# orybkin/video-gcp

Measured on AMD Instinct MI355X. Metric: predicted frames/sec, 64x64x3 seq_len=80 gcp_tree (posterior forward + all loss terms, model(inputs) and model.loss() of train.py:157-159, batch-stat BatchNorm), higher is better.
Workload: dtype f32 (encoder / decoder convs and the tree GEMMs from 512 rows: split-f16 MFMA with f32 accumulate, f32-equivalent; everything else exact f32 MFMA)

## Files before the change

### include/gcpx.h

```cpp
#ifndef GCPX_H
#define GCPX_H

#include <stdint.h>

#ifdef __cplusplus
extern "C" {
#endif

#define GCPX_VERSION 1

typedef enum gcpx_status {
    GCPX_OK = 0,
    GCPX_ERR_INVALID_ARG = -1,
    GCPX_ERR_UNSUPPORTED = -2,
    GCPX_ERR_HIP = -3,
    GCPX_ERR_COMM = -4
} gcpx_status;

typedef enum gcpx_act { GCPX_ACT_NONE = 0, GCPX_ACT_LRELU = 1, GCPX_ACT_TANH = 2 } gcpx_act;

int gcpx_version(void);
const char* gcpx_last_error(void);
int gcpx_conv_grid(void);

// ... 36 lines not shown
    const int32_t* raw_row_map;
    const int32_t* src_row_map;
    const int32_t* src_row_frames;
    int32_t n_src_rows;
    int32_t w_split_log2;
    const void* wpk_split;
    const int32_t* w_split_log2_dev;
    int32_t split_layout;
    int32_t nll_rows;
    const float* nll_target;
    float* nll_partial;
    const float* nll_row_weight;
    float nll_scale;
    int32_t _pad3;
    float* images_rows;
    int64_t images_rows_dup;
    const float* bwd_r;
    const float *bwd_scale, *bwd_shift, *bwd_mean, *bwd_rstd;
    const float* addend;
    int32_t addend_frame_div;
    int32_t _pad4;
} gcpx_conv_args;

typedef enum gcpx_split_layout { GCPX_SPLIT_PLAIN = 0, GCPX_SPLIT_ROWFOLD = 1, GCPX_SPLIT_HEAD32 = 2 } gcpx_split_layout;

int gcpx_conv3x3(const gcpx_conv_args* a, void* stream);
int gcpx_conv3x3_grid(const gcpx_conv_args* a);
int gcpx_conv4x4s2(const gcpx_conv_args* a, void* stream);
int gcpx_conv4x4s2_grid(void);
int gcpx_conv4x4s2_image(const float* x, const float* wpk, const float* bias, float* out,
                         int32_t F, int32_t Hin, int32_t Win, int32_t Cout, int32_t out_act, void* stream);

int gcpx_bn_finalize(const float* partial, int32_t n_partial, int32_t pitch, int32_t C, double count,
                     const float* gamma, const float* beta, float eps, float* scale, float* shift,
                     float* running_mean, float* running_var, float momentum, float* mean_out, float* rstd_out,
                     void* stream);
int gcpx_randn(float* out, int64_t n, uint64_t* state, void* stream);
int gcpx_bn_fold(const float* running_mean, const float* running_var, const float* gamma, const float* beta,
                 float eps, int32_t C, float* scale, float* shift, void* stream);

typedef struct gcpx_row_src {
    const float* ptr;
    const int32_t* rowidx;
    const float* scale;
    const float* shiftv;
    int64_t sb, sr;
    int32_t width;
// ... 510 lines not shown
```

### video-gcp_amd/csrc/conv3x3.hip

```cpp
#include "common.h"

#include <type_traits>

int gcpx_launch_up16_split(const gcpx_conv_args* a, hipStream_t stream, int grid);
int gcpx_launch_up32_split(const gcpx_conv_args* a, hipStream_t stream, int which, int grid);
int gcpx_launch_up16_fold(const gcpx_conv_args* a, hipStream_t stream, int grid);
int gcpx_launch_wave_split(const gcpx_conv_args* a, hipStream_t stream, int ct, int depth);

namespace {

template <int TILE> struct TileShape;
template <> struct TileShape<0> { static constexpr int TH = 8, TW = 32, TF = 1; };
template <> struct TileShape<1> { static constexpr int TH = 16, TW = 16, TF = 1; };
template <> struct TileShape<2> { static constexpr int TH = 8, TW = 8, TF = 4; };
template <> struct TileShape<3> { static constexpr int TH = 8, TW = 16, TF = 1; };

template <bool UP, int CC, int CT, int TILE>
struct ConvCfg {
    using TS = TileShape<TILE>;
    static constexpr int TH = TS::TH, TW = TS::TW, TF = TS::TF;
    static constexpr int RH = TH + 2, RW = TW + 2;
    static constexpr int LH = TH / 2 + 2, LW = TW / 2 + 2;
    static constexpr int CCP = (CC == 16) ? 24 : CC + 4;
    static constexpr int C4 = CC / 4;
    static constexpr int HI_FLOATS = TF * RH * RW * CCP;
    static constexpr int RAW_FLOATS = UP ? TF * LH * LW * CC : 0;
    static constexpr int RED_FLOATS = 4 * 2 * CT * 16;
    static constexpr int LDS_BYTES = (HI_FLOATS + RAW_FLOATS) * 4;
    static constexpr int PR = TH * TW * TF / 64;
// ... 1013 lines not shown
                red[(wave * 2 + 0) * 16 + q * 4 + r] = s1;
                red[(wave * 2 + 1) * 16 + q * 4 + r] = s2;
            }
        }
        __syncthreads();
        if (tid < 32) {
            const int which = tid >> 4, c = tid & 15;
            float sum = 0.f;
#pragma unroll
            for (int w = 0; w < 8; ++w) sum += red[(w * 2 + which) * 16 + c];
            a.stats_partial[((size_t)blockIdx.x * 2 + which) * 16 + c] = sum;
        }
    }
}

int launch_up16(const gcpx_conv_args* a, hipStream_t stream, bool query_only) {
    const int nchunk = a->Cin / 16;
    const int lds = UpWaveCfg::lds_bytes(nchunk);
    int grid = gcpx_conv_grid() / 2;
    const int nitems = a->F * (a->Hout / 4) * (a->Wout / 16);
    if (!a->stats_partial && grid * 8 > nitems) grid = (nitems + 7) / 8;
    if (query_only) return grid;
    if (a->wpk_split && a->split_layout == GCPX_SPLIT_ROWFOLD) return gcpx_launch_up16_fold(a, stream, grid);
    if (a->wpk_split) return gcpx_launch_up16_split(a, stream, grid);
    static int lds_set = 0;
    if (lds > lds_set) {
        hipError_t e = hipFuncSetAttribute(reinterpret_cast<const void*>(conv3x3_up16_kernel),
                                           hipFuncAttributeMaxDynamicSharedMemorySize, lds);
        if (e != hipSuccess) {
            gcpx_set_error("conv3x3 up16: hipFuncSetAttribute(%d B LDS): %s", lds, hipGetErrorString(e));
            return GCPX_ERR_HIP;
        }
        lds_set = lds;
    }
    const int ipw = (nitems + grid * 8 - 1) / (grid * 8);
    hipLaunchKernelGGL(conv3x3_up16_kernel, dim3(grid), dim3(512), lds, stream, *a, ipw, nitems);
    GCPX_CHECK_LAUNCH();
    return GCPX_OK;
}

int g_conv_grid = 0;

template <bool UP, int CC, int CT, int TILE>
int launch(const gcpx_conv_args* a, hipStream_t stream, bool query_only = false) {
    using Cfg = ConvCfg<UP, CC, CT, TILE>;
    if (a->Hout % Cfg::TH || a->Wout % Cfg::TW) {
// ... 40 lines not shown
int gcpx_launch_head_split(const gcpx_conv_args* a, hipStream_t stream);

static int conv3x3_dispatch(const gcpx_conv_args* a, hipStream_t stream, bool query_only) {
    GCPX_CHECK_ARG(a != nullptr, "null args");
    GCPX_CHECK_ARG(a->nsrc == 1 || a->nsrc == 2, "nsrc must be 1 or 2");
    GCPX_CHECK_ARG(a->src[0].C % 16 == 0 && (a->nsrc == 1 || a->src[1].C % 16 == 0), "source channels must be multiples of 16");
    const bool leading = !a->upsample && a->nsrc == 1 && a->Cin < a->src[0].C && a->Cin >= 32 && a->Cin % 16 == 0 && a->Cout == 16 && a->wpk_split &&
                         a->split_layout == GCPX_SPLIT_PLAIN && (!a->src_row_map || a->src_row_frames) && !getenv("GCPX_DGRAD_TILED");
    GCPX_CHECK_ARG(leading || a->Cin == a->src[0].C + (a->nsrc == 2 ? a->src[1].C : 0), "Cin != sum of sources");
    GCPX_CHECK_ARG(a->wpk && a->bias, "weights/bias missing");
    GCPX_CHECK_ARG(a->F > 0, "F <= 0");
    if (a->upsample) GCPX_CHECK_ARG(a->Hout == 2 * a->Hin && a->Wout == 2 * a->Win, "upsample: Hout != 2*Hin");
    else GCPX_CHECK_ARG(a->Hout == a->Hin && a->Wout == a->Win, "no upsample: Hout != Hin");
    const int CT = (a->Cout + 15) / 16;
    const bool need_out = a->head_mode == GCPX_HEAD_RAW || a->head_mode == GCPX_HEAD_DLM_BOTH;
    GCPX_CHECK_ARG(!need_out || a->out, "out is NULL");
    GCPX_CHECK_ARG(need_out || a->images, "images is NULL");
    GCPX_CHECK_ARG(!need_out || a->out_pitch % 4 == 0, "out_pitch % 4");
    GCPX_CHECK_ARG(!a->images_rows || (a->wpk_split && a->raw_row_map && a->images && a->Cout == 100 && !a->upsample &&
                                       (a->head_mode == GCPX_HEAD_DLM_MEAN || a->head_mode == GCPX_HEAD_DLM_BOTH ||
                                        a->head_mode == GCPX_HEAD_DLM_NLL || a->head_mode == GCPX_HEAD_DLM_NLL_GRAD)),
                   "images_rows: split-f16 mixture head with raw_row_map and images only");
    const int W = a->Wout;
    GCPX_CHECK_ARG(!a->addend || (a->upsample && a->addend_frame_div > 0 && a->wpk_split && a->Cout != 16),
                   "addend: split-f16 upsampling blocks with 32 / 64 output channels, addend_frame_div > 0");
    if (!a->upsample) {
        GCPX_CHECK_ARG(a->nsrc == 1 && a->src[0].frame_div == 1, "non-upsampling 3x3 conv takes one per-frame source");
        if (a->Cin == 16 && !a->src_row_map && W % 16 == 0 && a->Hout % 4 == 0) {
            if (a->Cout == 100) {
                GCPX_CHECK_ARG(!need_out || a->out_pitch >= 100, "mixture head: out_pitch < 100");
                GCPX_CHECK_ARG(a->head_mode != GCPX_HEAD_DLM_NLL || a->wpk_split, "GCPX_HEAD_DLM_NLL is built for the split-f16 head (wpk_split)");
                if (a->wpk_split) return query_only ? gcpx_conv_grid() / 2 : gcpx_launch_head_split(a, stream);
                return query_only ? gcpx_conv_grid() / 2 : launch_head<6, true>(a, stream);
            }
            if (CT == 1) return query_only ? gcpx_conv_grid() / 2 : launch_head<1, false>(a, stream);
        }
        GCPX_CHECK_ARG(a->head_mode == GCPX_HEAD_RAW && (!a->stats_partial || a->bwd_r), "plain 3x3 conv stores raw output, no statistics");
        if (a->bwd_r) {
            const bool fits = a->wpk_split && a->split_layout == GCPX_SPLIT_PLAIN && W % 16 == 0 && a->Hout % 4 == 0 && a->Cout == 16 &&
                              a->out_pitch == 16 && a->Cin >= 32 && a->Cin % 16 == 0 && (!a->src_row_map || a->src_row_frames) &&
                              a->stats_partial && a->bwd_scale && a->bwd_shift && a->bwd_mean && a->bwd_rstd && !getenv("GCPX_DGRAD_TILED");
            GCPX_CHECK_ARG(fits, "bwd_r: split-f16 plain 3x3 conv, 16 output channels at pitch 16, Cin >= 32, stats_partial and the four BatchNorm vectors");
        }
        static const bool tiled_only = getenv("GCPX_DGRAD_TILED") != nullptr;
        static const int depth = getenv("GCPX_DGRAD_DEPTH") ? atoi(getenv("GCPX_DGRAD_DEPTH")) : 2;
        GCPX_CHECK_ARG(!a->src_row_frames || (a->src_row_map && a->n_src_rows >= 0), "src_row_frames needs src_row_map and n_src_rows");
        if (!tiled_only && W % 16 == 0 && a->Hout % 4 == 0 && a->Cout == 16 && a->out_pitch % 4 == 0 && CT == 1 && a->Cin >= 32 &&
            (!a->src_row_map || a->src_row_frames) && WaveCfg<1>::lds_bytes(a->Cin / 16) <= 152 * 1024) {
// ... 8 lines not shown
        GCPX_CHECK_ARG(!leading, "Cin < src[0].C is built for the 16-output-channel wave kernel only (W % 16 == 0, H % 4 == 0)");
        static const bool wave32 = getenv("GCPX_DGRAD_NOWAVE32") == nullptr;
        if (wave32 && !tiled_only && W % 16 == 0 && a->Hout % 4 == 0 && a->Cout == 32 && a->out_pitch % 4 == 0 && a->Cin % 16 == 0 &&
            (!a->src_row_map || a->src_row_frames) && WaveCfg<2>::lds_bytes(a->Cin / 16) <= 152 * 1024) {
            if (query_only) return gcpx_conv_grid() / 2;
            if (a->wpk_split && a->split_layout == GCPX_SPLIT_PLAIN) {
                const int st = gcpx_launch_wave_split(a, stream, 2, 1);
                if (st != -1) return st;
            }
            return launch_wave<2, 1>(a, stream);
        }
        const int tile = W >= 32 ? 0 : (W == 16 ? 1 : (W == 8 ? 2 : -1));
#define GCPX_PLAIN(CC_, CT_)                                                            \
        do {                                                                            \
            if (tile == 0) return launch<false, CC_, CT_, 0>(a, stream, query_only);    \
            if (tile == 1) return launch<false, CC_, CT_, 1>(a, stream, query_only);    \
            if (tile == 2) return launch<false, CC_, CT_, 2>(a, stream, query_only);    \
        } while (0)
        if (a->Cin % 16 == 0 && CT == 4) GCPX_PLAIN(16, 4);
        if (a->Cin % 16 == 0 && CT == 2) GCPX_PLAIN(16, 2);
        if (a->Cin % 16 == 0 && CT == 1) GCPX_PLAIN(16, 1);
#undef GCPX_PLAIN
    } else {
        GCPX_CHECK_ARG(a->Cin % 32 == 0, "upsampling 3x3 conv expects Cin % 32 == 0");
        GCPX_CHECK_ARG(a->head_mode == GCPX_HEAD_RAW, "decoder blocks store raw output");
        if (a->Cout == 16) {
            GCPX_CHECK_ARG(W % 16 == 0 && a->Hout % 4 == 0 && a->out_pitch == 16 && a->Cin <= 64, "16-channel block shape");
            return launch_up16(a, stream, query_only);
        }
        if (a->wpk_split && !query_only && a->Cout == CT * 16 && a->out_pitch == a->Cout && a->out_act == GCPX_ACT_NONE) {
            if (W == 16 && CT == 2) return gcpx_launch_up32_split(a, stream, 0, launch<true, 32, 2, 1>(a, stream, true));
            if (W == 8 && CT == 2) return gcpx_launch_up32_split(a, stream, 1, launch<true, 32, 2, 2>(a, stream, true));
            if (W == 8 && CT == 4) return gcpx_launch_up32_split(a, stream, 2, launch<true, 32, 4, 2>(a, stream, true));
        }
        GCPX_CHECK_ARG(query_only || !a->addend, "addend: split-f16 upsampling blocks with 32 / 64 output channels only");
        if (W == 16 && CT == 2) return launch<true, 32, 2, 1>(a, stream, query_only);
        if (W == 8 && CT == 2) return launch<true, 32, 2, 2>(a, stream, query_only);
        if (W == 8 && CT == 4) return launch<true, 32, 4, 2>(a, stream, query_only);
    }
    gcpx_set_error("conv3x3: unsupported shape (up=%d Cin=%d Cout=%d W=%d)", a->upsample, a->Cin, a->Cout, W);
    return GCPX_ERR_UNSUPPORTED;
}

extern "C" int gcpx_conv3x3(const gcpx_conv_args* a, void* stream_) {
    return conv3x3_dispatch(a, reinterpret_cast<hipStream_t>(stream_), false);
}

// ... 2 lines not shown
```

### video-gcp_amd/csrc/conv3x3_split.hip

```cpp
#include "common.h"
#include "split_mfma.h"

#include <cstdlib>
#include <type_traits>

namespace {

struct SplitUpCfg {
    static constexpr int RW = 18, RH = 6, LW = 10, LH = 4, CC = 16, KS = 5;
    static constexpr int RAW_BYTES = LH * LW * CC * 4;
    static constexpr int PLANE_BYTES = RH * RW * 32;
    static constexpr int WAVE_BYTES = RAW_BYTES + 2 * PLANE_BYTES;
    static constexpr int NS = (LH * LW * 4 + 63) / 64;
    static constexpr int W_CHUNK_BYTES = KS * 2 * 1024;
    static int lds_bytes(int nchunk) { return nchunk * W_CHUNK_BYTES + 8 * WAVE_BYTES + 8 * 2 * 16 * 4; }
};

__global__ void __launch_bounds__(512, 2) conv3x3_up16_split_kernel(const gcpx_conv_args a, const int items_per_wave,
                                                                    const int nitems) {
    using Cfg = SplitUpCfg;
    constexpr int RW = Cfg::RW, RH = Cfg::RH, LW = Cfg::LW, LH = Cfg::LH, CC = Cfg::CC, NS = Cfg::NS, KS = Cfg::KS;
    extern __shared__ float4 smem4[];
    const int nchunk = a.Cin / CC;
    const char* wl = reinterpret_cast<const char*>(smem4);
// ... 748 lines not shown
    }
    if (optr) store_out();
    if (a.stats_partial) {
#pragma unroll
        for (int r = 0; r < 4; ++r) {
            const float s1 = row16_sum(st1[r]);
            const float s2 = row16_sum(st2[r]);
            if (j == 0) {
                red[(wave * 2 + 0) * 16 + q * 4 + r] = s1;
                red[(wave * 2 + 1) * 16 + q * 4 + r] = s2;
            }
        }
        __syncthreads();
        if (tid < 32) {
            const int which = tid >> 4, c = tid & 15;
            float sum = 0.f;
#pragma unroll
            for (int w = 0; w < 8; ++w) sum += red[(w * 2 + which) * 16 + c];
            a.stats_partial[((size_t)blockIdx.x * 2 + which) * 16 + c] = sum;
        }
    }
}

typedef unsigned int u32x4s __attribute__((ext_vector_type(4)));

template <int CT>
struct WaveSplitCfg {
    static constexpr int RW = 18, RH = 6, KS = 5;
    static constexpr int PLANE_BYTES = RH * RW * 32;
    static constexpr int REGION_BYTES = 2 * PLANE_BYTES;
    static constexpr int W_CHUNK_BYTES = KS * CT * 2 * 1024;
    static constexpr int NS = (RH * RW * 4 + 63) / 64;
    static int lds_bytes(int nchunk) { return nchunk * W_CHUNK_BYTES + 8 * REGION_BYTES + 256 + 1024; }
};

template <int CT, int DEPTH, bool ACTB = false>
__global__ void __launch_bounds__(512, 2) conv3x3_wave_split_kernel(const gcpx_conv_args a, const int nitems) {
    using Cfg = WaveSplitCfg<CT>;
    constexpr int RW = Cfg::RW, RH = Cfg::RH, NS = Cfg::NS, KS = Cfg::KS;
    extern __shared__ float4 smem4[];
    const int nchunk = a.Cin / 16;
    const char* wl = reinterpret_cast<const char*>(smem4);
    const int tid = threadIdx.x, lane = tid & 63;
    const int wave = __builtin_amdgcn_readfirstlane(tid >> 6);
    char* reg = reinterpret_cast<char*>(smem4) + nchunk * Cfg::W_CHUNK_BYTES + wave * Cfg::REGION_BYTES;
    const int j = lane & 15, q = lane >> 4;
// ... 347 lines not shown
    GCPX_CHECK_ARG(a->Cin == 32 && a->Cout == 16 && a->Hin % Cfg::R == 0 && a->Hout == 2 * a->Hin && a->Wout == 2 * a->Win && a->Wout % 16 == 0,
                   "row-folded block: 32 -> 16 channels, Hin a multiple of 4, output width a multiple of 16");
    GCPX_CHECK_ARG(a->src[0].C % 4 == 0 && (a->nsrc == 1 ? a->src[0].C == 32 : a->src[0].C + a->src[1].C == 32), "source channels");
    static const bool prio = getenv("GCPX_FOLD_NOPRIO") == nullptr;
    auto kern = prio ? conv3x3_up16_fold_kernel<true> : conv3x3_up16_fold_kernel<false>;
    static bool attr_set = false;
    if (!attr_set) {
        for (auto k : {conv3x3_up16_fold_kernel<true>, conv3x3_up16_fold_kernel<false>}) {
            hipError_t e = hipFuncSetAttribute(reinterpret_cast<const void*>(k), hipFuncAttributeMaxDynamicSharedMemorySize, Cfg::LDS_BYTES);
            if (e != hipSuccess) {
                gcpx_set_error("conv3x3 row-folded up16: hipFuncSetAttribute(%d B LDS): %s", Cfg::LDS_BYTES, hipGetErrorString(e));
                return GCPX_ERR_HIP;
            }
        }
        attr_set = true;
    }
    const int nitems = a->F * (a->Hin / Cfg::R) * (a->Wout / 16);
    const int ipw = (nitems + grid * 8 - 1) / (grid * 8);
    hipLaunchKernelGGL(kern, dim3(grid), dim3(512), Cfg::LDS_BYTES, stream, *a, ipw, nitems);
    GCPX_CHECK_LAUNCH();
    return GCPX_OK;
}

extern "C" int gcpx_fold_upsample_weights(const float* w, int32_t Cout, int32_t Cin, float* out, void* stream_) {
    GCPX_CHECK_ARG(w && out && Cout > 0 && Cin > 0, "bad arguments");
    const int n = 24 * Cout * Cin;
    hipLaunchKernelGGL(fold_up_weights_kernel, dim3((n + 255) / 256), dim3(256), 0, reinterpret_cast<hipStream_t>(stream_), w, Cout, Cin, out);
    GCPX_CHECK_LAUNCH();
    return GCPX_OK;
}

int gcpx_launch_wave_split(const gcpx_conv_args* a, hipStream_t stream, int ct, int depth) {
    const int nchunk = a->Cin / 16;
    if (ct == 1) {
        if (WaveSplitCfg<1>::lds_bytes(nchunk) > 160 * 1024) return -1;
        if (a->bwd_r) {
            static const int d = getenv("GCPX_WAVE_DEPTH") ? atoi(getenv("GCPX_WAVE_DEPTH")) : 1;
            return d == 3 ? launch_wave_split_t<1, 3, true>(a, stream) : d == 2 ? launch_wave_split_t<1, 2, true>(a, stream) : launch_wave_split_t<1, 1, true>(a, stream);
        }
        return depth == 2 ? launch_wave_split_t<1, 2>(a, stream) : launch_wave_split_t<1, 1>(a, stream);
    }
    if (WaveSplitCfg<2>::lds_bytes(nchunk) > 160 * 1024) return -1;
    return launch_wave_split_t<2, 1>(a, stream);
}
```

### video-gcp_amd/forward_plan.py

```python
import ctypes as C
import os
from contextlib import contextmanager

import torch

from . import packing as pk
from . import runtime as rt
from .hparams import GCPHParams
from .params import init_params, encoder_layers, encoder_skip_layers, decoder_layers
from .plan_ops import _Plan, _addr, N_LANES


class ForwardPlanMixin:

    def _plan_encoder(self, plan, tag, x_ptr, F, out_ptr, out_ob, out_orow, out_rpb):
        hp, P, lib = self._hp, self.pk, self.lib
        G = lib.gcpx_conv4x4s2_grid()
        S = hp.img_sz
        skip_idx = encoder_skip_layers(hp)
        skips = {}
        a0 = self._buf(f"{tag}.a0", (F, S // 2, S // 2, hp.ngf))
        enc_rec = dict(F=F, x_ptr=x_ptr, a0=a0, r={}, out=(out_ptr, out_ob, out_orow, out_rpb))
        plan.rec[f"enc:{tag}"] = enc_rec
        plan.add(f"enc.input:{tag}", lib.gcpx_conv4x4s2_image, x_ptr, P["enc.input.w"].data_ptr(),
# ... 70 lines not shown
    def _plan_decoder_features(self, plan, e_src, F, rpb, skips):
        hp, P, lib = self._hp, self.pk, self.lib
        ctop = self._c_top
        d0 = self._buf("dec.d0", (F, 4, 4, ctop))
        plan.rec["dec"] = dict(F=F, rpb=rpb, e_src=e_src, d0=d0, blocks=[], skips=skips)
        nrb = lib.gcpx_gemm_row_blocks(F, 16 * ctop)
        st = self._buf("dec.st0", (nrb, 2, 16 * ctop)) if self.training else None
        self._gemm(plan, "dec.input", [e_src], F, 16 * ctop, rpb, P["dec.input.w"], P["dec.input.b"], out=d0.data_ptr(),
                   ob=rpb * 16 * ctop, orow=16 * ctop, stats=st)
        sc, sh = self._bn(plan, "dec.bn0", "decoder.net.input.norm", ctop, st, nrb, 16 * ctop, F * 16)
        prev = (d0.data_ptr(), ctop, 1, sc, sh, rt.ACT_LRELU)
        res = 4
        for name, c_prev, c_skip, skip_idx, cout in decoder_layers(hp):
            srcs = [prev]
            if skip_idx >= 0:
                t, C_, ssc, ssh, sact = skips[skip_idx]
                assert C_ == c_skip and t.shape[1] == res
                srcs.append((t.data_ptr(), C_, rpb, ssc, ssh, sact))
            o = self._buf(f"dec.{name}", (F, 2 * res, 2 * res, cout))
            cpad = (cout + 15) // 16 * 16
            hoist = (skip_idx >= 0 and rpb > 1 and F % rpb == 0 and self.split_f16 and cout in (32, 64) and c_prev % 32 == 0 and
                     c_skip % 32 == 0 and f"dec.{name}" in self.pk_split and "fold" not in self.pk_split[f"dec.{name}"] and
                     os.environ.get("GCPX_NO_SKIP_HOIST") is None)
            addend = None
            if hoist:
                addend = self._buf(f"dec.{name}.skip", (F // rpb, 2 * res, 2 * res, cout))
                t, C_, ssc, ssh, sact = skips[skip_idx]
                zb = self._buf(f"dec.{name}.zero_bias", (cpad,), zero=True)
                a_s = self._conv_args([(t.data_ptr(), C_, 1, ssc, ssh, sact)], F // rpb, res, res, 2 * res, 2 * res, cout, cout,
                                      P[f"dec.{name}.w"], zb, addend, upsample=1)
                self._set_split(a_s, f"dec.{name}")
                a_s.wpk_split = a_s.wpk_split + (c_prev // 32) * 9 * (cpad // 16) * 2048
                plan.keep.append(a_s)
                plan.add(f"dec.{name}.skip", lib.gcpx_conv3x3, C.byref(a_s))
                srcs_main = [prev]
            else:
                srcs_main = srcs
            a = self._conv_args(srcs_main, F, res, res, 2 * res, 2 * res, cout, cout, P[f"dec.{name}.w"], P[f"dec.{name}.b"],
                                o, upsample=1, stats=(o if self.training else None))
            if hoist:
                a.addend, a.addend_frame_div = addend.data_ptr(), rpb
            self._set_split(a, f"dec.{name}")
            Gl = lib.gcpx_conv3x3_grid(C.byref(a))
            assert Gl > 0, rt.lib().gcpx_last_error()
            st = self._buf(f"dec.st.{name}", (Gl, 2, cpad)) if self.training else None
            a.stats_partial = st.data_ptr() if st is not None else None
            plan.keep.append(a)
            plan.add(f"dec.{name}", lib.gcpx_conv3x3, C.byref(a))
            plan.rec["dec"]["blocks"].append(dict(name=name, srcs=srcs, out=o, res_in=res, cout=cout, c_prev=c_prev, c_skip=c_skip,
                                                  skip_idx=skip_idx))
            res *= 2
            sc, sh = self._bn(plan, f"dec.bn.{name}", f"decoder.net.{name}.norm", cout, st, Gl, cpad, F * res * res)
            prev = (o.data_ptr(), cout, 1, sc, sh, rt.ACT_LRELU)
        assert res == hp.img_sz
        return prev

    def _build_plan(self, key, tin):
        hp, P, lib = self._hp, self.pk, self.lib
        B, has_traj, has_z, sample_prior, phase = key[0], key[1], key[2], key[3], key[4]
        pred_len = key[9]
        train_aux = has_traj and phase == "train" and not sample_prior
        L, T, N = hp.hierarchy_levels, hp.max_seq_len, hp.n_nodes
        nz, nv, H, SD = hp.nz_enc, hp.nz_vae, hp.nz_mid_lstm, hp.lstm_state_dim
        PS = 2 ** L + 1
        plan = _Plan(lib)
# ... 463 lines not shown
```

### video-gcp_amd/packing.py

```python
import torch

_LANE = torch.arange(64)
_LI = _LANE % 16
_LQ = _LANE // 16


def _pad_rows(w, rows):
    if w.shape[0] == rows:
        return w
    pad = torch.zeros((rows - w.shape[0],) + tuple(w.shape[1:]), dtype=w.dtype, device=w.device)
    return torch.cat([w, pad], 0)


def pack_gemm(w):
    N, K = w.shape
    assert K % 16 == 0, (N, K)
    NT = (N + 15) // 16
    w = _pad_rows(w, NT * 16)
    dev = w.device
    kg = torch.arange(K // 16, device=dev)[:, None, None, None]
    nt = torch.arange(NT, device=dev)[None, :, None, None]
    li = _LI.to(dev)[None, None, :, None]
    lq = _LQ.to(dev)[None, None, :, None]
    s = torch.arange(4, device=dev)[None, None, None, :]
# ... 297 lines not shown
    return torch.stack(out, 0).float()


def conv3x3_fold_gather(fw):
    assert fw.shape == (24, 16, 32)
    dev = fw.device
    t = torch.arange(24, device=dev)[:, None, None]
    li = _LI.to(dev)[None, :, None]
    lq = _LQ.to(dev)[None, :, None]
    el = torch.arange(8, device=dev)[None, None, :]
    return fw[t, li, lq * 8 + el].contiguous()


def pack_conv3x3_fold(w):
    w1, w2, e = split_f16(conv3x3_fold_gather(fold_up_weights(w)))
    return torch.stack([w1, w2], 1).contiguous().view(torch.int16), e


def conv3x3_fold_index():
    ids = torch.arange(24 * 16 * 32, dtype=torch.float64).view(24, 16, 32)
    return conv3x3_fold_gather(ids).reshape(-1).to(torch.int32)


def lstm_gate_interleave(w_ih, w_hh, b_ih, b_hh):
    H = w_hh.shape[1]
    w = torch.cat([w_ih, w_hh], dim=1)
    K = w.shape[1]
    w = w.view(4, H, K).permute(1, 0, 2).reshape(4 * H, K)
    b = (b_ih + b_hh).view(4, H).t().reshape(4 * H)
    return w.contiguous(), b.contiguous()
```

### video-gcp_amd/runtime.py

```python
import ctypes as C
import os

_HERE = os.path.dirname(os.path.abspath(__file__))
LIB_PATH = os.path.join(_HERE, "libgcpx.so")

ACT_NONE, ACT_LRELU, ACT_TANH = 0, 1, 2
HEAD_RAW, HEAD_DLM_MEAN, HEAD_DLM_BOTH, HEAD_TANH_NCHW, HEAD_DLM_NLL, HEAD_DLM_NLL_GRAD = 0, 1, 2, 3, 4, 5
SPLIT_PLAIN, SPLIT_ROWFOLD, SPLIT_HEAD32 = 0, 1, 2
EPI_NONE, EPI_LRELU, EPI_LSTM, EPI_GAUSS_SAMPLE = 0, 1, 2, 3
MLP_PLAIN, MLP_GAUSS, MLP_TANH = 0, 1, 2

vp = C.c_void_p
i32 = C.c_int32
i64 = C.c_int64


class ConvSrc(C.Structure):
    _fields_ = [("ptr", vp), ("scale", vp), ("shift", vp), ("C", i32), ("frame_div", i32), ("act", i32), ("_pad", i32)]


class ConvArgs(C.Structure):
    _fields_ = [("src", ConvSrc * 2), ("nsrc", i32), ("F", i32), ("Hin", i32), ("Win", i32), ("Hout", i32),
                ("Wout", i32), ("Cin", i32), ("Cout", i32), ("out_pitch", i32), ("upsample", i32), ("out_act", i32),
                ("head_mode", i32), ("wpk", vp), ("bias", vp), ("out", vp), ("images", vp), ("stats_partial", vp),
                ("raw_row_map", vp), ("src_row_map", vp), ("src_row_frames", vp), ("n_src_rows", i32), ("w_split_log2", i32), ("wpk_split", vp), ("w_split_log2_dev", vp),
                ("split_layout", i32), ("nll_rows", i32), ("nll_target", vp), ("nll_partial", vp), ("nll_row_weight", vp),
                ("nll_scale", C.c_float), ("_pad3", i32), ("images_rows", vp), ("images_rows_dup", i64), ("bwd_r", vp), ("bwd_scale", vp), ("bwd_shift", vp), ("bwd_mean", vp),
                ("bwd_rstd", vp), ("addend", vp), ("addend_frame_div", i32), ("_pad4", i32)]


class LossArgs(C.Structure):
# ... 281 lines not shown
```

### video-gcp_amd/weights.py

```python
import ctypes as C
import os
from contextlib import contextmanager

import torch

from . import packing as pk
from . import runtime as rt
from .hparams import GCPHParams
from .params import init_params, encoder_layers, encoder_skip_layers, decoder_layers
from .plan_ops import _addr


class WeightsMixin:

    def _flatten_params(self, params):
        off, self._poff = 0, {}
        for k, v in params.items():
            self._poff[k] = (off, tuple(v.shape))
            off += (v.numel() + 3) // 4 * 4
        self.theta = torch.zeros(off, dtype=torch.float32, device=self.device)
        self.sd = {}
        for k, v in params.items():
            o, shp = self._poff[k]
            view = self.theta[o:o + v.numel()].view(shp)
# ... 21 lines not shown
            d["gn_b"] = torch.stack([sd[f"{prefix}.pyramid-{i}.norm.bias"] for i in range(n_mid)]).contiguous()
        d["w_out"] = pk.pack_gemm(sd[f"{prefix}.head.linear.weight"])
        d["b_out"] = pk.pad_vec(sd[f"{prefix}.head.linear.bias"], out_pad)
        return d

    def _pack_all(self):
        if self._arena is not None:
            self.repack()
            return
        self.pk = self._pack_tree(self.sd)
        if self._hp.tree_lstm:
            self._pack_fused_embed()
        self._pack_split()
        self._pack_gemm_split()

    def _pack_split(self):
        self.pk_split = {}
        hp = self._hp
        todo = []
        if hp.decoder_distribution == "discrete_logistic_mixture":
            todo.append(("dec.head", "decoder.gen_head.conv.weight", pk.dlm_channel_perm(hp.n_mixtures)))
            if self.head32 and hp.n_mixtures == 10 and hp.head_channels == 100:
                todo.append(("dec.head32", "decoder.gen_head.conv.weight", ("head32", pk.dlm_channel_perm(hp.n_mixtures))))
        for name, c_prev, c_skip, skip_idx, cout in decoder_layers(hp):
            if cout == 16 and c_prev + c_skip == 32:
                todo.append((f"dec.{name}", f"decoder.net.{name}.conv.weight", "rowfold"))
            elif cout == 16:
                todo.append((f"dec.{name}", f"decoder.net.{name}.conv.weight", None))
            elif cout in (32, 64) and (c_prev + c_skip) % 32 == 0:
                todo.append((f"dec.{name}", f"decoder.net.{name}.conv.weight", "tiled32"))
        for name, cin, cout, norm in self._enc_layers[1:]:
            if cin == 16 or cin % 32 == 0:
                todo.append((f"enc.{name}", f"encoder.net.{name}.conv.weight", "enc4x4"))
        for name, key, perm in todo:
            off, shp = self._poff[key]
            d = {}
            if perm == "enc4x4":
                idx = pk.conv4x4_split_index(shp, off).to(self.device)
            elif perm == "rowfold":
                d["fold"] = torch.zeros(24 * shp[0] * shp[1], dtype=torch.float32, device=self.device)
                d["fold_src"] = (off, shp[0], shp[1])
                idx = pk.conv3x3_fold_index().to(self.device)
            elif perm == "tiled32":
                idx = pk.conv3x3_split32_index(shp, off).to(self.device)
            elif isinstance(perm, tuple) and perm[0] == "head32":
                idx = pk.head32_index(shp, off, perm[1]).to(self.device)
            else:
                idx = pk.conv3x3_split_index(shp, off, perm).to(self.device)
            d.update(idx=idx, out=torch.zeros(2 * idx.numel(), dtype=torch.int16, device=self.device),
                     log2=torch.zeros(1, dtype=torch.int32, device=self.device))
            self.pk_split[name] = d
        self.repack_split()

    def repack_split(self, stream=None):
        st = stream if stream is not None else torch.cuda.current_stream(self.device).cuda_stream
        if not self.pk_split:
            return
        tab = self._split_tab
        key = (self.theta.data_ptr(),) + tuple((d["out"].data_ptr(), d["idx"].data_ptr()) for d in self.pk_split.values())
        if tab is None or tab[2] != key:
            descs = []
            for name, d in self.pk_split.items():
                src = d["fold"] if "fold" in d else self.theta
                e = rt.SplitPackDesc()
                e.src, e.idx, e.out, e.log2_out, e.n = src.data_ptr(), d["idx"].data_ptr(), d["out"].data_ptr(), d["log2"].data_ptr(), d["idx"].numel()
                descs.append(e)
            arr = (rt.SplitPackDesc * len(descs))(*descs)
            dev = torch.frombuffer(bytearray(bytes(arr)), dtype=torch.uint8).to(self.device)
            tab = self._split_tab = (dev, len(descs), key, torch.zeros(len(descs), dtype=torch.int32, device=self.device))
        for name, d in self.pk_split.items():
            if "fold_src" in d:
                off, cout, cin = d["fold_src"]
                rt.check(self.lib.gcpx_fold_upsample_weights(self.theta.data_ptr() + 4 * off, cout, cin, d["fold"].data_ptr(), st), "fold_upsample_weights")
        rt.check(self.lib.gcpx_split_pack_group2(tab[0].data_ptr(), tab[1], tab[3].data_ptr(), st), "split_pack_group2")
# ... 8 lines not shown
        for name, W in self.pk.items():
            if not (isinstance(W, dict) and name.startswith("tree")):
                continue
            for key, wpk in W.items():
                if not (key.endswith(".w") and (key.startswith("lstm") or key == "proj.w")):
                    continue
                stack = wpk if wpk.dim() == 5 else wpk[None]
                if (stack.shape[2] * 16) % 64 or (stack.shape[1] * 16) % 64:
                    continue
                packs = [pk.pack_gemm_split(pk.unpack_gemm(w, w.shape[1] * 16)) for w in stack]
                ws = torch.stack([p_[0] for p_ in packs]).contiguous().to(self.device)
                es = torch.tensor([p_[1] for p_ in packs], dtype=torch.int32, device=self.device)
                self._gsplit[wpk.data_ptr()] = (ws, es)

    def _set_split(self, a, name):
        d = self.pk_split.get(name)
        layout = None
        if name == "dec.head" and self.head32 and a.head_mode in (rt.HEAD_DLM_MEAN, rt.HEAD_DLM_NLL, rt.HEAD_DLM_NLL_GRAD) \
                and "dec.head32" in self.pk_split:
            d, layout = self.pk_split["dec.head32"], rt.SPLIT_HEAD32
        if self.split_f16 and d is not None:
            a.wpk_split, a.w_split_log2_dev = d["out"].data_ptr(), d["log2"].data_ptr()
            if layout is None:
                layout = rt.SPLIT_ROWFOLD if "fold" in d else rt.SPLIT_PLAIN
            a.split_layout = layout

    def _pack_fused_embed(self):
        hp = self._hp
        for l in range(hp.hierarchy_levels if hp.untied_layers else 1):
            p = f"tree_module.tree_modules.{l}.subgoal_pred"
            sd = self.sd
            We, be = sd[f"{p}.embed.weight"].double(), sd[f"{p}.embed.bias"].double()
            Wih = sd[f"{p}.lstm.0.weight_ih"].double()
            Wf = (Wih @ We).float()
            bf = (Wih @ be).float() + sd[f"{p}.lstm.0.bias_ih"]
            w, b = pk.lstm_gate_interleave(Wf, sd[f"{p}.lstm.0.weight_hh"], bf, sd[f"{p}.lstm.0.bias_hh"])
            self.pk[f"tree{l}"]["lstm0f.w"], self.pk[f"tree{l}"]["lstm0f.b"] = pk.pack_gemm(w), b

    def _pack_tree(self, sd):
        hp = self._hp
        self._psd = sd
        P = {}
        layers, c_top = encoder_layers(hp)
        self._enc_layers, self._c_top = layers, c_top
        P["enc.input.w"] = pk.pack_conv4x4_image(sd["encoder.net.input.conv.weight"])
        P["enc.input.b"] = sd["encoder.net.input.conv.bias"].contiguous()
        for name, cin, cout, norm in layers[1:]:
# ... 209 lines not shown
```

Baseline: 504,900.

## Hoist skip-branch conv for 16-channel decoder block into per-sequence addend

Extends the skip-hoisting trick to the 16-in/16-skip/16-out upsampling decoder block. The skip input is shared across frames of a sequence, so its half of the conv is computed once per sequence into an addend buffer. The main conv then runs only over the 16 previous-layer channels using a new row-folded split-f16 kernel with 16-channel input. This removes redundant per-frame work on the skip half, at the cost of a new specialized kernel, extra weight packs and an extra launch.

```diff
diff --git a/include/gcpx.h b/include/gcpx.h
--- a/include/gcpx.h
+++ b/include/gcpx.h
@@ -82,7 +82,7 @@
     int32_t _pad4;
 } gcpx_conv_args;
 
-typedef enum gcpx_split_layout { GCPX_SPLIT_PLAIN = 0, GCPX_SPLIT_ROWFOLD = 1, GCPX_SPLIT_HEAD32 = 2 } gcpx_split_layout;
+typedef enum gcpx_split_layout { GCPX_SPLIT_PLAIN = 0, GCPX_SPLIT_ROWFOLD = 1, GCPX_SPLIT_HEAD32 = 2, GCPX_SPLIT_ROWFOLD16 = 3 } gcpx_split_layout;
 
 int gcpx_conv3x3(const gcpx_conv_args* a, void* stream);
 int gcpx_conv3x3_grid(const gcpx_conv_args* a);
diff --git a/video-gcp_amd/csrc/conv3x3.hip b/video-gcp_amd/csrc/conv3x3.hip
--- a/video-gcp_amd/csrc/conv3x3.hip
+++ b/video-gcp_amd/csrc/conv3x3.hip
@@ -5,6 +5,7 @@
 int gcpx_launch_up16_split(const gcpx_conv_args* a, hipStream_t stream, int grid);
 int gcpx_launch_up32_split(const gcpx_conv_args* a, hipStream_t stream, int which, int grid);
 int gcpx_launch_up16_fold(const gcpx_conv_args* a, hipStream_t stream, int grid);
+int gcpx_launch_up16_fold16(const gcpx_conv_args* a, hipStream_t stream, int grid);
 int gcpx_launch_wave_split(const gcpx_conv_args* a, hipStream_t stream, int ct, int depth);
 
 namespace {
@@ -1064,6 +1065,7 @@
     if (!a->stats_partial && grid * 8 > nitems) grid = (nitems + 7) / 8;
     if (query_only) return grid;
     if (a->wpk_split && a->split_layout == GCPX_SPLIT_ROWFOLD) return gcpx_launch_up16_fold(a, stream, grid);
+    if (a->wpk_split && a->split_layout == GCPX_SPLIT_ROWFOLD16) return gcpx_launch_up16_fold16(a, stream, grid);
     if (a->wpk_split) return gcpx_launch_up16_split(a, stream, grid);
     static int lds_set = 0;
     if (lds > lds_set) {
@@ -1150,8 +1152,8 @@
                                         a->head_mode == GCPX_HEAD_DLM_NLL || a->head_mode == GCPX_HEAD_DLM_NLL_GRAD)),
                    "images_rows: split-f16 mixture head with raw_row_map and images only");
     const int W = a->Wout;
-    GCPX_CHECK_ARG(!a->addend || (a->upsample && a->addend_frame_div > 0 && a->wpk_split && a->Cout != 16),
-                   "addend: split-f16 upsampling blocks with 32 / 64 output channels, addend_frame_div > 0");
+    GCPX_CHECK_ARG(!a->addend || (a->upsample && a->addend_frame_div > 0 && a->wpk_split && (a->Cout != 16 || a->split_layout == GCPX_SPLIT_ROWFOLD16)),
+                   "addend: split-f16 upsampling blocks (32 / 64 output channels, or the 16-channel row-folded block), addend_frame_div > 0");
     if (!a->upsample) {
         GCPX_CHECK_ARG(a->nsrc == 1 && a->src[0].frame_div == 1, "non-upsampling 3x3 conv takes one per-frame source");
         if (a->Cin == 16 && !a->src_row_map && W % 16 == 0 && a->Hout % 4 == 0) {
@@ -1206,7 +1208,8 @@
         if (a->Cin % 16 == 0 && CT == 1) GCPX_PLAIN(16, 1);
 #undef GCPX_PLAIN
     } else {
-        GCPX_CHECK_ARG(a->Cin % 32 == 0, "upsampling 3x3 conv expects Cin % 32 == 0");
+        GCPX_CHECK_ARG(a->Cin % 32 == 0 || (a->Cin == 16 && a->wpk_split && a->split_layout == GCPX_SPLIT_ROWFOLD16),
+                       "upsampling 3x3 conv expects Cin % 32 == 0 (16 channels: the row-folded split-f16 block, GCPX_SPLIT_ROWFOLD16)");
         GCPX_CHECK_ARG(a->head_mode == GCPX_HEAD_RAW, "decoder blocks store raw output");
         if (a->Cout == 16) {
             GCPX_CHECK_ARG(W % 16 == 0 && a->Hout % 4 == 0 && a->out_pitch == 16 && a->Cin <= 64, "16-channel block shape");
diff --git a/video-gcp_amd/csrc/conv3x3_split.hip b/video-gcp_amd/csrc/conv3x3_split.hip
--- a/video-gcp_amd/csrc/conv3x3_split.hip
+++ b/video-gcp_amd/csrc/conv3x3_split.hip
@@ -794,6 +794,261 @@
     }
 }
 
+struct Fold16Cfg {
+    static constexpr int R = 4;
+    static constexpr int PR = R + 2, PW = 10, RW = 18, CC = 16;
+    static constexpr int RAW_BYTES = PR * PW * CC * 4;
+    static constexpr int PLANE_BYTES = PR * RW * 32;
+    static constexpr int WAVE_BYTES = 2 * PLANE_BYTES;
+    static constexpr int NT = 16;
+    static constexpr int W_BYTES = NT * 2048;
+    static constexpr int LDS_BYTES = W_BYTES + 8 * WAVE_BYTES + 8 * 2 * 16 * 4 + 3 * 16 * 4;
+    static constexpr int NS = (PR * PW * 4 + 63) / 64;
+    static constexpr int NO = (PR * RW * 4 + 63) / 64;
+};
+
+__global__ void __launch_bounds__(512, 2) conv3x3_up16_fold16_kernel(const gcpx_conv_args a, const int items_per_wave, const int nitems) {
+    using Cfg = Fold16Cfg;
+    constexpr int R = Cfg::R, PR = Cfg::PR, PW = Cfg::PW, RW = Cfg::RW, NS = Cfg::NS, NO = Cfg::NO;
+    extern __shared__ float4 smem4[];
+    const char* wl = reinterpret_cast<const char*>(smem4);
+    const int tid = threadIdx.x, lane = tid & 63;
+    const int wave = __builtin_amdgcn_readfirstlane(tid >> 6);
+    char* wbuf = reinterpret_cast<char*>(smem4) + Cfg::W_BYTES + wave * Cfg::WAVE_BYTES;
+    float* red = reinterpret_cast<float*>(reinterpret_cast<char*>(smem4) + Cfg::W_BYTES + 8 * Cfg::WAVE_BYTES);
+    float* biasl = red + 8 * 2 * 16;
+    const int j = lane & 15, q = lane >> 4;
+    const int H = a.Hout, W = a.Wout, Hin = a.Hin, Win = a.Win;
+    const int ncb = W / 16, nrb = Hin / R;
+
+    for (int i = tid; i < Cfg::W_BYTES / 16; i += 512) smem4[i] = reinterpret_cast<const float4*>(a.wpk_split)[i];
+    if (tid < 16) {
+        biasl[tid] = a.bias[tid];
+        biasl[16 + tid] = a.src[0].scale ? a.src[0].scale[tid] : 1.f;
+        biasl[32 + tid] = a.src[0].scale ? a.src[0].shift[tid] : 0.f;
+    }
+    __syncthreads();
+
+    const int c4 = lane & 3, ps = lane >> 2;
+    const float* sptr = a.src[0].ptr;
+    const int srcC = a.src[0].C;
+    const float slope = a.src[0].act == GCPX_ACT_LRELU ? 0.2f : 1.f;
+    const int fdiv0 = a.src[0].frame_div;
+    const int ew = a.w_split_log2_dev ? __builtin_amdgcn_readfirstlane(*a.w_split_log2_dev) : a.w_split_log2;
+    const float4 bv = *reinterpret_cast<const float4*>(a.bias + q * 4);
+
+    const int gw = blockIdx.x * 8 + wave;
+    const int item0 = gw * items_per_wave;
+    const int item_end = min(item0 + items_per_wave, nitems);
+    const float* const addend = a.addend;
+    const int div = addend ? a.addend_frame_div : 1;
+    auto origin = [&](int it, int& run, int& f, int& y0, int& x0) {
+        run = it / div;
+        const int rb = run % nrb;
+        const int t = run / nrb;
+        y0 = rb * R; x0 = (t % ncb) * 16;
+        f = (t / ncb) * div + (it - run * div);
+    };
+    const int rowM = ps >> 3, colM = ps & 7;
+    const int rowL = ps >> 1, colL = 8 + (ps & 1);
+    const int WinC = Win * srcC;
+    const int raw_wr_m = (rowM * PW + colM) * 64 + c4 * 16;
+    const int raw_wr_l = (rowL * PW + colL) * 64 + c4 * 16;
+    const int raw_rd_m = (ps >> 1) * 64 + c4 * 16;
+    const int raw_rd_l = (rowL * PW + 8) * 64 + c4 * 16;
+    const int reg_wr_m = ps * 32 + c4 * 8;
+    const int reg_wr_l = (rowL * RW + 16 + (ps & 1)) * 32 + c4 * 8;
+    const float wa_m = (ps & 1) ? 0.25f : 0.75f;
+    float4 pre[2][NS];
+    auto issue_loads = [&](int it, float4 (&dst)[NS]) __attribute__((always_inline)) {
+        int run, f, y0, x0;
+        origin(it, run, f, y0, x0);
+        const float* base = sptr + (size_t)(f / fdiv0) * Hin * Win * srcC;
+        const int ly0 = y0 - 1, lx0 = x0 / 2 - 1;
+        const int sxm = min(max(lx0 + colM, 0), Win - 1) * srcC + c4 * 4;
+        const int sxl = min(max(lx0 + colL, 0), Win - 1) * srcC + c4 * 4;
+#pragma unroll
+        for (int k = 0; k < NS - 1; ++k) {
+            const int sy = min(max(ly0 + 2 * k + rowM, 0), Hin - 1);
+            dst[k] = *reinterpret_cast<const float4*>(base + (unsigned)(sy * WinC + sxm));
+        }
+        dst[NS - 1] = *reinterpret_cast<const float4*>(base + (unsigned)(min(max(ly0 + rowL, 0), Hin - 1) * WinC + sxl));
+    };
+
+    f32x4 ab[R][2];
+#pragma unroll
+    for (int yi = 0; yi < R; ++yi) { ab[yi][0] = f32x4{bv.x, bv.y, bv.z, bv.w}; ab[yi][1] = ab[yi][0]; }
+    int ab_run = -1;
+
+    f32x4 st1 = f32x4{0, 0, 0, 0}, st2 = f32x4{0, 0, 0, 0};
+    if (item0 < item_end) {
+        issue_loads(item0, pre[0]);
+        issue_loads(min(item0 + 1, item_end - 1), pre[1]);
+    }
+    __builtin_amdgcn_s_waitcnt(0x0f70);
+
+    const int boff0 = (j + (q >> 1)) * 32 + (q & 1) * 16, boff1 = (j + 2) * 32 + (q & 1) * 16;
+
+    auto do_item = [&](const int item, float4 (&pre)[NS]) __attribute__((always_inline)) {
+        int run, f, y0, x0;
+        origin(item, run, f, y0, x0);
+        const bool top = (y0 == 0), bot = (y0 + R == Hin), lft = (x0 == 0), rgt = (x0 + 16 == W);
+
+        if (addend && run != ab_run) {
+            ab_run = run;
+            const float* adp = addend + (((size_t)(f / div) * H + 2 * y0) * W + x0) * 16;
+            const float4 bl = *reinterpret_cast<const float4*>(biasl + q * 4);
+#pragma unroll
+            for (int yi = 0; yi < R; ++yi)
+#pragma unroll
+                for (int py = 0; py < 2; ++py) {
+                    const float4 ad = *reinterpret_cast<const float4*>(adp + (unsigned)((2 * yi + py) * W * 16 + j * 16 + q * 4));
+                    ab[yi][py] = f32x4{ad.x + bl.x, ad.y + bl.y, ad.z + bl.z, ad.w + bl.w};
+                }
+        }
+
+        float amax = 0.f;
+        const float4 bn_s = *reinterpret_cast<const float4*>(biasl + 16 + c4 * 4), bn_t = *reinterpret_cast<const float4*>(biasl + 32 + c4 * 4);
+#pragma unroll
+        for (int k = 0; k < NS; ++k) {
+            float4 v = pre[k];
+            v.x = fmaf(v.x, bn_s.x, bn_t.x); v.y = fmaf(v.y, bn_s.y, bn_t.y); v.z = fmaf(v.z, bn_s.z, bn_t.z); v.w = fmaf(v.w, bn_s.w, bn_t.w);
+            v.x = fmaxf(v.x, v.x * slope); v.y = fmaxf(v.y, v.y * slope); v.z = fmaxf(v.z, v.z * slope); v.w = fmaxf(v.w, v.w * slope);
+            char* dst = wbuf + (k < NS - 1 ? raw_wr_m + k * 2 * PW * 64 : raw_wr_l);
+            if (k < NS - 1 || lane < 48) *reinterpret_cast<float4*>(dst) = v;
+            else v = make_float4(0.f, 0.f, 0.f, 0.f);
+            amax = fmaxf(amax, fmaxf(fmaxf(fabsf(v.x), fabsf(v.y)), fmaxf(fabsf(v.z), fabsf(v.w))));
+        }
+        issue_loads(min(item + 2, item_end - 1), pre);
+        amax = wave_max_nonneg(amax);
+        int ex = 14 + 127 - (int)((__float_as_uint(amax) >> 23) & 0xff);
+        ex = __builtin_amdgcn_readfirstlane(amax > 0.f ? max(-100, min(min(100, 126 - ew), ex)) : min(100, 126 - ew));
+        const float sx2 = __uint_as_float((unsigned)(127 + ex) << 23);
+
+        h4 o1[NO], o2[NO];
+        const float sc_first = (lft && ps == 0) ? 0.f : sx2;
+        const float sc_last = (rgt && (ps & 1)) ? 0.f : sx2;
+#pragma unroll
+        for (int k = 0; k < NO; ++k) {
+            const char* rp = wbuf + (k < NO - 1 ? raw_rd_m + k * PW * 64 : raw_rd_l);
+            const float4 A = *reinterpret_cast<const float4*>(rp);
+            const float4 B = *reinterpret_cast<const float4*>(rp + 64);
+            const float sc = k < NO - 1 ? sc_first : sc_last;
+            const float wa = wa_m * sc, wb = (1.f - wa_m) * sc;
+            float4 v;
+            v.x = fmaf(wa, A.x, wb * B.x); v.y = fmaf(wa, A.y, wb * B.y); v.z = fmaf(wa, A.z, wb * B.z); v.w = fmaf(wa, A.w, wb * B.w);
+            h4 p1, p2;
+            p1[0] = (_Float16)v.x; p1[1] = (_Float16)v.y; p1[2] = (_Float16)v.z; p1[3] = (_Float16)v.w;
+            p2[0] = (_Float16)fmaf((float)p1[0], -1.f, v.x); p2[1] = (_Float16)fmaf((float)p1[1], -1.f, v.y);
+            p2[2] = (_Float16)fmaf((float)p1[2], -1.f, v.z); p2[3] = (_Float16)fmaf((float)p1[3], -1.f, v.w);
+            o1[k] = p1;
+            o2[k] = p2;
+        }
+        __builtin_amdgcn_fence(__ATOMIC_ACQ_REL, "wavefront");
+        __builtin_amdgcn_wave_barrier();
+#pragma unroll
+        for (int k = 0; k < NO; ++k) {
+            char* dst = wbuf + (k < NO - 1 ? reg_wr_m + k * RW * 32 : reg_wr_l);
+            if (k < NO - 1 || lane < 48) {
+                *reinterpret_cast<h4*>(dst) = o1[k];
+                *reinterpret_cast<h4*>(dst + Cfg::PLANE_BYTES) = o2[k];
+            }
+        }
+
+        f32x4 acc[R][2];
+#pragma unroll
+        for (int yi = 0; yi < R; ++yi) { acc[yi][0] = f32x4{0, 0, 0, 0}; acc[yi][1] = f32x4{0, 0, 0, 0}; }
+        auto load_w = [&](const int t, h8 (&w)[2]) __attribute__((always_inline)) {
+            const char* wp = wl + t * 2048 + lane * 16;
+            w[0] = *reinterpret_cast<const h8*>(wp);
+            w[1] = *reinterpret_cast<const h8*>(wp + 1024);
+        };
+        auto load_b = [&](const int kind, const int r, h8 (&b)[2]) __attribute__((always_inline)) {
+            const char* bp = wbuf + r * RW * 32 + (kind ? boff1 : boff0);
+            b[0] = *reinterpret_cast<const h8*>(bp);
+            b[1] = *reinterpret_cast<const h8*>(bp + Cfg::PLANE_BYTES);
+        };
+        h8 wq[2][2], bq[2][PR][2], wc[2];
+        load_w(0, wq[0]);
+#pragma unroll
+        for (int r = 0; r < 4; ++r) load_b(0, r, bq[0][r]);
+        __builtin_amdgcn_s_setprio(1);
+        static_for<0, 12>([&](auto tc) __attribute__((always_inline)) {
+            constexpr int t = decltype(tc)::value, kind = t / 6, blk = t % 6, dyl = blk / 2, py = blk % 2;
+            constexpr bool more = t + 1 < 12;
+            constexpr bool pre_next = blk >= 2 && kind + 1 < 2;
+            constexpr bool pre_own = blk < 2;
+            if constexpr (more) {
+                constexpr int t1 = t + 1, kind1 = t1 / 6, blk1 = t1 % 6;
+                load_w((blk1 % 2) * 6 + (blk1 / 2) * 2 + kind1, wq[t1 & 1]);
+            }
+            if constexpr (pre_next) load_b(kind + 1, blk - 2, bq[(kind + 1) & 1][blk - 2]);
+            if constexpr (pre_own) load_b(kind, 4 + blk, bq[kind & 1][4 + blk]);
+            const h8 w1 = wq[t & 1][0], w2 = wq[t & 1][1];
+#pragma unroll
+            for (int yi = 0; yi < R; ++yi) acc[yi][py] = mfma32h(w2, bq[kind & 1][yi + dyl][0], acc[yi][py]);
+#pragma unroll
+            for (int yi = 0; yi < R; ++yi) acc[yi][py] = mfma32h(w1, bq[kind & 1][yi + dyl][1], acc[yi][py]);
+#pragma unroll
+            for (int yi = 0; yi < R; ++yi) acc[yi][py] = mfma32h(w1, bq[kind & 1][yi + dyl][0], acc[yi][py]);
+            __builtin_amdgcn_sched_group_barrier(0x100, (more ? 2 : 0) + ((pre_next || pre_own) ? 2 : 0), 0);
+            __builtin_amdgcn_sched_group_barrier(0x008, 12, 0);
+            if constexpr (blk == 5) {
+                if (top) {
+                    load_w(12 + kind, wc);
+                    acc[0][0] = mfma32h(wc[1], bq[kind & 1][0][0], acc[0][0]);
+                    acc[0][0] = mfma32h(wc[0], bq[kind & 1][0][1], acc[0][0]);
+                    acc[0][0] = mfma32h(wc[0], bq[kind & 1][0][0], acc[0][0]);
+                }
+                if (bot) {
+                    load_w(14 + kind, wc);
+                    acc[R - 1][1] = mfma32h(wc[1], bq[kind & 1][PR - 1][0], acc[R - 1][1]);
+                    acc[R - 1][1] = mfma32h(wc[0], bq[kind & 1][PR - 1][1], acc[R - 1][1]);
+                    acc[R - 1][1] = mfma32h(wc[0], bq[kind & 1][PR - 1][0], acc[R - 1][1]);
+                }
+            }
+        });
+        __builtin_amdgcn_s_setprio(0);
+
+        const float inv = __uint_as_float((unsigned)(127 - ex - ew) << 23);
+        float* optr = a.out + (((size_t)f * H + 2 * y0) * W + x0) * 16;
+#pragma unroll
+        for (int yi = 0; yi < R; ++yi)
+#pragma unroll
+            for (int py = 0; py < 2; ++py) {
+                f32x4 v = acc[yi][py];
+                const f32x4 t = ab[yi][py];
+                v[0] = fmaf(v[0], inv, t[0]); v[1] = fmaf(v[1], inv, t[1]); v[2] = fmaf(v[2], inv, t[2]); v[3] = fmaf(v[3], inv, t[3]);
+                *reinterpret_cast<float4*>(optr + (unsigned)((2 * yi + py) * W * 16 + j * 16 + q * 4)) = make_float4(v[0], v[1], v[2], v[3]);
+                st1 += v;
+                st2 += v * v;
+            }
+    };
+    for (int item = item0; item < item_end; item += 2) {
+        do_item(item, pre[0]);
+        if (item + 1 < item_end) do_item(item + 1, pre[1]);
+    }
+    if (a.stats_partial) {
+#pragma unroll
+        for (int r = 0; r < 4; ++r) {
+            const float s1 = row16_sum(st1[r]);
+            const float s2 = row16_sum(st2[r]);
+            if (j == 0) {
+                red[(wave * 2 + 0) * 16 + q * 4 + r] = s1;
+                red[(wave * 2 + 1) * 16 + q * 4 + r] = s2;
+            }
+        }
+        __syncthreads();
+        if (tid < 32) {
+            const int which = tid >> 4, c = tid & 15;
+            float sum = 0.f;
+#pragma unroll
+            for (int w = 0; w < 8; ++w) sum += red[(w * 2 + which) * 16 + c];
+            a.stats_partial[((size_t)blockIdx.x * 2 + which) * 16 + c] = sum;
+        }
+    }
+}
+
 typedef unsigned int u32x4s __attribute__((ext_vector_type(4)));
 
 template <int CT>
@@ -1187,6 +1442,30 @@
     return GCPX_OK;
 }
 
+int gcpx_launch_up16_fold16(const gcpx_conv_args* a, hipStream_t stream, int grid) {
+    using Cfg = Fold16Cfg;
+    GCPX_CHECK_ARG(a->Cin == 16 && a->Cout == 16 && a->nsrc == 1 && a->src[0].C == 16 && a->Hin % Cfg::R == 0 && a->Hout == 2 * a->Hin &&
+                   a->Wout == 2 * a->Win && a->Wout % 16 == 0,
+                   "row-folded 16-channel block: one 16-channel source, 16 output channels, Hin a multiple of 4, output width a multiple of 16");
+    GCPX_CHECK_ARG(!a->addend || (a->addend_frame_div > 0 && a->F % a->addend_frame_div == 0),
+                   "row-folded 16-channel block: F must be a multiple of addend_frame_div (items are walked sequence by sequence)");
+    auto kern = conv3x3_up16_fold16_kernel;
+    static bool attr_set = false;
+    if (!attr_set) {
+        hipError_t e = hipFuncSetAttribute(reinterpret_cast<const void*>(kern), hipFuncAttributeMaxDynamicSharedMemorySize, Cfg::LDS_BYTES);
+        if (e != hipSuccess) {
+            gcpx_set_error("conv3x3 row-folded up16 (16 channels): hipFuncSetAttribute(%d B LDS): %s", Cfg::LDS_BYTES, hipGetErrorString(e));
+            return GCPX_ERR_HIP;
+        }
+        attr_set = true;
+    }
+    const int nitems = a->F * (a->Hin / Cfg::R) * (a->Wout / 16);
+    const int ipw = (nitems + grid * 8 - 1) / (grid * 8);
+    hipLaunchKernelGGL(kern, dim3(grid), dim3(512), Cfg::LDS_BYTES, stream, *a, ipw, nitems);
+    GCPX_CHECK_LAUNCH();
+    return GCPX_OK;
+}
+
 extern "C" int gcpx_fold_upsample_weights(const float* w, int32_t Cout, int32_t Cin, float* out, void* stream_) {
     GCPX_CHECK_ARG(w && out && Cout > 0 && Cin > 0, "bad arguments");
     const int n = 24 * Cout * Cin;
diff --git a/video-gcp_amd/forward_plan.py b/video-gcp_amd/forward_plan.py
--- a/video-gcp_amd/forward_plan.py
+++ b/video-gcp_amd/forward_plan.py
@@ -116,15 +116,20 @@
             hoist = (skip_idx >= 0 and rpb > 1 and F % rpb == 0 and self.split_f16 and cout in (32, 64) and c_prev % 32 == 0 and
                      c_skip % 32 == 0 and f"dec.{name}" in self.pk_split and "fold" not in self.pk_split[f"dec.{name}"] and
                      os.environ.get("GCPX_NO_SKIP_HOIST") is None)
+            hoist16 = (skip_idx >= 0 and rpb > 1 and F % rpb == 0 and self.split_f16 and cout == 16 and c_prev == 16 and c_skip == 16 and
+                       f"dec.{name}.f16a" in self.pk_split and res % 4 == 0 and os.environ.get("GCPX_NO_SKIP_HOIST") is None)
             addend = None
-            if hoist:
+            if hoist or hoist16:
                 addend = self._buf(f"dec.{name}.skip", (F // rpb, 2 * res, 2 * res, cout))
                 t, C_, ssc, ssh, sact = skips[skip_idx]
                 zb = self._buf(f"dec.{name}.zero_bias", (cpad,), zero=True)
                 a_s = self._conv_args([(t.data_ptr(), C_, 1, ssc, ssh, sact)], F // rpb, res, res, 2 * res, 2 * res, cout, cout,
                                       P[f"dec.{name}.w"], zb, addend, upsample=1)
-                self._set_split(a_s, f"dec.{name}")
-                a_s.wpk_split = a_s.wpk_split + (c_prev // 32) * 9 * (cpad // 16) * 2048
+                if hoist16:
+                    self._set_split(a_s, f"dec.{name}.f16b")
+                else:
+                    self._set_split(a_s, f"dec.{name}")
+                    a_s.wpk_split = a_s.wpk_split + (c_prev // 32) * 9 * (cpad // 16) * 2048
                 plan.keep.append(a_s)
                 plan.add(f"dec.{name}.skip", lib.gcpx_conv3x3, C.byref(a_s))
                 srcs_main = [prev]
@@ -132,9 +137,9 @@
                 srcs_main = srcs
             a = self._conv_args(srcs_main, F, res, res, 2 * res, 2 * res, cout, cout, P[f"dec.{name}.w"], P[f"dec.{name}.b"],
                                 o, upsample=1, stats=(o if self.training else None))
-            if hoist:
+            if hoist or hoist16:
                 a.addend, a.addend_frame_div = addend.data_ptr(), rpb
-            self._set_split(a, f"dec.{name}")
+            self._set_split(a, f"dec.{name}.f16a" if hoist16 else f"dec.{name}")
             Gl = lib.gcpx_conv3x3_grid(C.byref(a))
             assert Gl > 0, rt.lib().gcpx_last_error()
             st = self._buf(f"dec.st.{name}", (Gl, 2, cpad)) if self.training else None
diff --git a/video-gcp_amd/packing.py b/video-gcp_amd/packing.py
--- a/video-gcp_amd/packing.py
+++ b/video-gcp_amd/packing.py
@@ -343,6 +343,31 @@
     return conv3x3_fold_gather(ids).reshape(-1).to(torch.int32)
 
 
+def conv3x3_fold16_gather(fw, cbase=0):
+    assert fw.shape[0] == 24 and fw.shape[1] == 16 and fw.shape[2] >= cbase + 16
+    dev = fw.device
+    bases = [py * 9 + dyl * 3 for py in range(2) for dyl in range(3)] + [18, 21]
+    fz = torch.cat([fw, torch.zeros((1,) + tuple(fw.shape[1:]), dtype=fw.dtype, device=dev)], 0)
+    li, lq = _LI.to(dev)[:, None], _LQ.to(dev)[:, None]
+    el = torch.arange(8, device=dev)[None, :]
+    frags = []
+    for b in bases:
+        for kind in range(2):
+            tset = (b + lq // 2) if kind == 0 else torch.where(lq // 2 == 0, torch.full_like(lq, b + 2), torch.full_like(lq, 24))
+            frags.append(fz[tset, li, cbase + 8 * (lq % 2) + el])
+    return torch.stack(frags, 0).contiguous()
+
+
+def pack_conv3x3_fold16(w, cbase=0):
+    w1, w2, e = split_f16(conv3x3_fold16_gather(fold_up_weights(w), cbase))
+    return torch.stack([w1, w2], 1).contiguous().view(torch.int16), e
+
+
+def conv3x3_fold16_index(cin, cbase):
+    ids = (torch.arange(24 * 16 * cin, dtype=torch.float64) + 1).view(24, 16, cin)
+    return (conv3x3_fold16_gather(ids, cbase).reshape(-1) - 1).to(torch.int32)
+
+
 def lstm_gate_interleave(w_ih, w_hh, b_ih, b_hh):
     H = w_hh.shape[1]
     w = torch.cat([w_ih, w_hh], dim=1)
diff --git a/video-gcp_amd/runtime.py b/video-gcp_amd/runtime.py
--- a/video-gcp_amd/runtime.py
+++ b/video-gcp_amd/runtime.py
@@ -6,7 +6,7 @@
 
 ACT_NONE, ACT_LRELU, ACT_TANH = 0, 1, 2
 HEAD_RAW, HEAD_DLM_MEAN, HEAD_DLM_BOTH, HEAD_TANH_NCHW, HEAD_DLM_NLL, HEAD_DLM_NLL_GRAD = 0, 1, 2, 3, 4, 5
-SPLIT_PLAIN, SPLIT_ROWFOLD, SPLIT_HEAD32 = 0, 1, 2
+SPLIT_PLAIN, SPLIT_ROWFOLD, SPLIT_HEAD32, SPLIT_ROWFOLD16 = 0, 1, 2, 3
 EPI_NONE, EPI_LRELU, EPI_LSTM, EPI_GAUSS_SAMPLE = 0, 1, 2, 3
 MLP_PLAIN, MLP_GAUSS, MLP_TANH = 0, 1, 2
 
diff --git a/video-gcp_amd/weights.py b/video-gcp_amd/weights.py
--- a/video-gcp_amd/weights.py
+++ b/video-gcp_amd/weights.py
@@ -67,9 +67,12 @@
             todo.append(("dec.head", "decoder.gen_head.conv.weight", pk.dlm_channel_perm(hp.n_mixtures)))
             if self.head32 and hp.n_mixtures == 10 and hp.head_channels == 100:
                 todo.append(("dec.head32", "decoder.gen_head.conv.weight", ("head32", pk.dlm_channel_perm(hp.n_mixtures))))
+        hoist16 = set()
         for name, c_prev, c_skip, skip_idx, cout in decoder_layers(hp):
             if cout == 16 and c_prev + c_skip == 32:
                 todo.append((f"dec.{name}", f"decoder.net.{name}.conv.weight", "rowfold"))
+                if self.split_f16 and skip_idx >= 0 and c_prev == 16 and c_skip == 16 and os.environ.get("GCPX_NO_SKIP_HOIST") is None:
+                    hoist16.add(f"dec.{name}")
             elif cout == 16:
                 todo.append((f"dec.{name}", f"decoder.net.{name}.conv.weight", None))
             elif cout in (32, 64) and (c_prev + c_skip) % 32 == 0:
@@ -95,6 +98,12 @@
             d.update(idx=idx, out=torch.zeros(2 * idx.numel(), dtype=torch.int16, device=self.device),
                      log2=torch.zeros(1, dtype=torch.int32, device=self.device))
             self.pk_split[name] = d
+            if perm == "rowfold" and name in hoist16:
+                for tag, cbase in (("f16a", 0), ("f16b", 16)):
+                    i16 = pk.conv3x3_fold16_index(shp[1], cbase).to(self.device)
+                    self.pk_split[f"{name}.{tag}"] = dict(fold=d["fold"], fold16=True, idx=i16,
+                                                          out=torch.zeros(2 * i16.numel(), dtype=torch.int16, device=self.device),
+                                                          log2=torch.zeros(1, dtype=torch.int32, device=self.device))
         self.repack_split()
 
     def repack_split(self, stream=None):
@@ -149,7 +158,7 @@
         if self.split_f16 and d is not None:
             a.wpk_split, a.w_split_log2_dev = d["out"].data_ptr(), d["log2"].data_ptr()
             if layout is None:
-                layout = rt.SPLIT_ROWFOLD if "fold" in d else rt.SPLIT_PLAIN
+                layout = rt.SPLIT_ROWFOLD16 if d.get("fold16") else (rt.SPLIT_ROWFOLD if "fold" in d else rt.SPLIT_PLAIN)
             a.split_layout = layout
 
     def _pack_fused_embed(self):
```

Measured after the change: 514,800 (median of 6 runs). +2.0%, better.
